# ZulutionAI/MoviiGen1.1

Measured on AMD Instinct MI355X. Metric: denoise-steps/sec, higher is better.
Workload: dtype bf16; 1 GPU; 14B T2V 1920x832x81f bf16 (the metric's configuration; BASELINE configs[2] shape); layers=40, parallelism=single, solver=unipc, weights=random N(0,0.02) bf16, seed 0

## Files before the change

### moviigen1.1_amd/csrc/attn_hd128.hip

```cpp
#include "common.h"
#include "../../include/moviigen_hip.h"

#define ATT_QB 256

__global__ __launch_bounds__(256) void pack_kv_kernel(const uint16_t* __restrict__ k, int64_t ldk,
                                                      const uint16_t* __restrict__ v, int64_t ldv, int64_t L,
                                                      uint16_t* __restrict__ kp, uint16_t* __restrict__ vp, int nt,
                                                      int korder) {
    __shared__ uint16_t tile[64][128 + 8];
    const int head = blockIdx.y, t = blockIdx.x;
    const int64_t k0 = (int64_t)t * 64;
    const int64_t tbase = ((int64_t)head * nt + t) * 8192;
    if (k) {
#pragma unroll
        for (int i = 0; i < 4; ++i) {
            const int id = threadIdx.x + i * 256;
            const int r = id >> 4, c = id & 15;
            u16x8_t u = {0, 0, 0, 0, 0, 0, 0, 0};
            if (k0 + r < L) u = *(const u16x8_t*)(k + (k0 + r) * ldk + head * 128 + c * 8);
            const int row = korder ? ((r & 32) | ((r & 4) << 2) | ((r & 24) >> 1) | (r & 3)) : r;
            *(u16x8_t*)(kp + tbase + c * 512 + row * 8) = u;
        }
    }
    if (v) {
#pragma unroll
        for (int i = 0; i < 4; ++i) {
            const int id = threadIdx.x + i * 256;
            const int r = id >> 4, c = id & 15;
            u16x8_t u = {0, 0, 0, 0, 0, 0, 0, 0};
            if (k0 + r < L) u = *(const u16x8_t*)(v + (k0 + r) * ldv + head * 128 + c * 8);
            *(u16x8_t*)&tile[r][c * 8] = u;
        }
        __syncthreads();
#pragma unroll
        for (int i = 0; i < 4; ++i) {
            const int id = threadIdx.x + i * 256;
            const int kc = id >> 7, d = id & 127;
            u16x8_t u;
#pragma unroll
            for (int j = 0; j < 8; ++j) u[j] = tile[kc * 8 + j][d];
            *(u16x8_t*)(vp + tbase + kc * 1024 + d * 8) = u;
        }
    }
}

#ifdef MG_AB_BUILD
int mg_attn_w64_launch(const uint16_t* q, int64_t ldq, const uint16_t* kp, const uint16_t* vp, uint16_t* o, int64_t ldo,
                       int64_t Lq, int64_t Lk, int heads, float c_log2, int nqb, float* lse, hipStream_t st);
#endif
int mg_attn_m16_launch(const uint16_t* q, int64_t ldq, const uint16_t* kp, const uint16_t* vp, uint16_t* o, int64_t ldo,
                       int64_t Lq, int64_t Lk, int heads, float c_log2, int prescaled, int nqb, float* lse, int reserve_cus,
                       unsigned* workspace, hipStream_t st);

#ifdef MG_AB_BUILD
static int g_attn_variant = 0;
extern "C" int mg_attn_set_variant(int v) {
    if (v != 0 && v != 3) return MG_ERR_ARG;
    g_attn_variant = v;
    return MG_OK;
}
#else
static constexpr int g_attn_variant = 0;
#endif

extern "C" int mg_pack_kv_bf16(const uint16_t* k, int64_t ldk, const uint16_t* v, int64_t ldv, int64_t L, int heads,
                               int head_dim, uint16_t* kp, uint16_t* vp, void* stream) {
    if ((!k && !v) || (k && !kp) || (v && !vp)) return MG_ERR_ARG;
    if (head_dim != 128 || heads <= 0 || L <= 0 || (k && (ldk & 7)) || (v && (ldv & 7))) return MG_ERR_SHAPE;
    const int nt = (int)((L + 63) / 64);
    hipLaunchKernelGGL(pack_kv_kernel, dim3(nt, heads), dim3(256), 0, (hipStream_t)stream, k, ldk, v, ldv, L, kp, vp,
                       nt, g_attn_variant == 3 ? 0 : 1);
    return mg_check_launch();
}

static int attn_fwd_impl(const uint16_t* q, int64_t ldq, const uint16_t* kp, const uint16_t* vp, uint16_t* o, int64_t ldo,
                         float* lse, int64_t Lq, int64_t Lk, int heads, float scale, int prescaled, int reserve_cus, void* workspace,
                         void* stream) {
    if (!q || !kp || !vp || !o) return MG_ERR_ARG;
    if ((uintptr_t)workspace & 7) return MG_ERR_SHAPE;
    if (Lq < 0 || Lk <= 0 || heads <= 0 || reserve_cus < 0) return MG_ERR_SHAPE;
    if ((ldq & 7) || (ldo & 3)) return MG_ERR_SHAPE;
    if (((uintptr_t)q & 15) || ((uintptr_t)kp & 15) || ((uintptr_t)vp & 15) || ((uintptr_t)o & 7)) return MG_ERR_SHAPE;
    if (Lq == 0) return MG_OK;
    const int64_t nqb64 = (Lq + ATT_QB - 1) / ATT_QB;
    if (nqb64 * heads > 0x7fffffffLL) return MG_ERR_SHAPE;
    const int nqb = (int)nqb64;
    const float c_log2 = scale * 1.4426950408889634f;
    hipStream_t st = (hipStream_t)stream;
#ifdef MG_AB_BUILD
    if (g_attn_variant == 3)
        return mg_attn_w64_launch(q, ldq, kp, vp, o, ldo, Lq, Lk, heads, prescaled ? 1.0f : c_log2, nqb, lse, st);
#endif
    return mg_attn_m16_launch(q, ldq, kp, vp, o, ldo, Lq, Lk, heads, c_log2, prescaled, nqb, lse, reserve_cus, (unsigned*)workspace, st);
}

extern "C" int64_t mg_attn_workspace_bytes(void) { return 256; }

extern "C" int mg_attn_fwd_bf16_hd128_lse(const uint16_t* q, int64_t ldq, const uint16_t* kp, const uint16_t* vp,
                                          uint16_t* o, int64_t ldo, float* lse, int64_t Lq, int64_t Lk, int heads,
                                          float scale, void* workspace, void* stream) {
    return attn_fwd_impl(q, ldq, kp, vp, o, ldo, lse, Lq, Lk, heads, scale, 0, 0, workspace, stream);
}
extern "C" int mg_attn_fwd_bf16_hd128(const uint16_t* q, int64_t ldq, const uint16_t* kp, const uint16_t* vp,
                                      uint16_t* o, int64_t ldo, int64_t Lq, int64_t Lk, int heads, float scale,
                                      void* workspace, void* stream) {
    return attn_fwd_impl(q, ldq, kp, vp, o, ldo, nullptr, Lq, Lk, heads, scale, 0, 0, workspace, stream);
}
extern "C" int mg_attn_fwd_bf16_hd128_prescaled(const uint16_t* q, int64_t ldq, const uint16_t* kp, const uint16_t* vp,
                                                uint16_t* o, int64_t ldo, float* lse, int64_t Lq, int64_t Lk, int heads,
                                                int reserve_cus, void* workspace, void* stream) {
    return attn_fwd_impl(q, ldq, kp, vp, o, ldo, lse, Lq, Lk, heads, 1.0f, 1, reserve_cus, workspace, stream);
}
```

### moviigen1.1_amd/csrc/attn_hd128_w64.hip

```cpp
#include <type_traits>
#include "common.h"
#include "../../include/moviigen_hip.h"

#define W64_THREADS 256
#define W64_QB 256
#define W64_TILE 16384
#define W64_K(slot) ((slot) * W64_TILE)
#define W64_V(slot) (3 * W64_TILE + (slot) * W64_TILE)

MG_DEV bf16x8_t w64_bf(u32x4_t v) { return __builtin_bit_cast(bf16x8_t, v); }

struct W64State {
    f32x16_t ot[4][2];
    f32x16_t st[2][2];
    bf16x8_t pf[2][2][2];
    float m_run[2], l_run[2];
    int bad;
};

template <int OFF>
MG_DEV void w64_rd(bf16x8_t& dst, unsigned addr) {
    asm volatile("ds_read_b128 %0, %1 offset:%2" : "=v"(dst) : "v"(addr), "i"(OFF));
}
template <int N>
MG_DEV void w64_wait() {
    asm volatile("s_waitcnt lgkmcnt(%0)" ::"i"(N) : "memory");
}
MG_DEV void w64_mfma_s0(f32x16_t& acc, const bf16x8_t& a, const bf16x8_t& b) {
    asm volatile("v_mfma_f32_32x32x16_bf16 %0, %1, %2, 0" : "=&v"(acc) : "v"(a), "v"(b));
}
MG_DEV void w64_mfma_s(f32x16_t& acc, const bf16x8_t& a, const bf16x8_t& b) {
    asm volatile("v_mfma_f32_32x32x16_bf16 %0, %1, %2, %0" : "+v"(acc) : "v"(a), "v"(b));
}
MG_DEV void w64_mfma_s_after_valu(f32x16_t& acc, const bf16x8_t& a, const bf16x8_t& b) {
    asm volatile("s_nop 7\n\ts_nop 7\n\tv_mfma_f32_32x32x16_bf16 %0, %1, %2, %0" : "+v"(acc) : "v"(a), "v"(b));
}
constexpr int w64_koff(int i) { return i * 2048; }
constexpr int w64_voff(int i) { return (i >> 2) * 4096 + (i & 3) * 512; }

template <int KB>
MG_DEV void w64_softmax_exact(W64State& s, float c_log2) {
#pragma unroll
    for (int qb = 0; qb < 2; ++qb) {
        float tmax = s.st[KB][qb][0];
#pragma unroll
        for (int r = 1; r < 16; ++r) tmax = fmaxf(tmax, s.st[KB][qb][r]);
        tmax = fmaxf(tmax, __shfl_xor(tmax, 32, 64));
        const float m_new = fmaxf(s.m_run[qb], tmax);
        const float mc = m_new * c_log2;
        float psum = 0.f;
        float p[16];
#pragma unroll
        for (int r = 0; r < 16; ++r) {
            p[r] = __builtin_amdgcn_exp2f(s.st[KB][qb][r] * c_log2 - mc);
            psum += p[r];
        }
#pragma unroll
        for (int h = 0; h < 2; ++h) {
            u32x4_t w;
#pragma unroll
            for (int e = 0; e < 4; ++e) w[e] = pack_bf2(p[h * 8 + 2 * e], p[h * 8 + 2 * e + 1]);
            s.pf[KB][qb][h] = w64_bf(w);
        }
        const float alpha = __builtin_amdgcn_exp2f((s.m_run[qb] - m_new) * c_log2);
        s.l_run[qb] = s.l_run[qb] * alpha + psum;
#pragma unroll
        for (int d = 0; d < 4; ++d)
#pragma unroll
            for (int e = 0; e < 16; ++e) s.ot[d][qb][e] *= alpha;
        s.m_run[qb] = m_new;
    }
}

template <int KB>
MG_DEV void w64_mask_init(W64State& s, int lim, int g) {
#pragma unroll
    for (int qb = 0; qb < 2; ++qb)
#pragma unroll
        for (int r = 0; r < 16; ++r) {
            const int key = KB * 32 + (r >> 3) * 16 + g * 8 + (r & 7);
            s.st[KB][qb][r] = key >= lim ? -1e30f : 0.f;
        }
}

template <int KB, int SMODE, bool PV, bool SM, typename Dma>
MG_DEV void w64_step(W64State& s, const bf16x8_t (&qf)[2][8], bf16x8_t (&kf)[4], bf16x8_t (&vf)[4], unsigned lds_k,
                     unsigned lds_v, unsigned nk, unsigned nv, float c_log2, Dma dma) {
    constexpr int SB = 1 - KB;
#ifndef W64_PK_ADD
#define W64_PK_ADD 0
#endif
    float mc[2], psa[2] = {0.f, 0.f}, psb[2] = {0.f, 0.f};
    f32x2_t ps2[2] = {{0.f, 0.f}, {0.f, 0.f}};
    u32x4_t w[2][2];
    if (SM) {
        mc[0] = s.m_run[0] * c_log2;
        mc[1] = s.m_run[1] * c_log2;
    }
    float pa = 0.f, pb = 0.f;
    auto pair_a = [&](int i, int half) __attribute__((always_inline)) {
        if (SM) {
            const int qb = i >> 2, j = (i & 3) * 2 + half;
            pa = __builtin_amdgcn_exp2f(s.st[SB][qb][2 * j] * c_log2 - mc[qb]);
            pb = __builtin_amdgcn_exp2f(s.st[SB][qb][2 * j + 1] * c_log2 - mc[qb]);
            asm volatile("" : "+v"(pa), "+v"(pb));
        }
    };
    auto pair_b = [&](int i, int half) __attribute__((always_inline)) {
        if (SM) {
            const int qb = i >> 2, j = (i & 3) * 2 + half;
#if W64_PK_ADD
            asm volatile("v_pk_add_f32 %0, %0, %1" : "+v"(ps2[qb]) : "v"(__builtin_shufflevector((f32x2_t){pa, pa}, (f32x2_t){pb, pb}, 0, 2)));
            unsigned pk = pack_bf2(pa, pb);
            asm volatile("" : "+v"(pk));
#else
            psa[qb] += pa;
            psb[qb] += pb;
            unsigned pk = pack_bf2(pa, pb);
            asm volatile("" : "+v"(pk), "+v"(psa[qb]), "+v"(psb[qb]));
#endif
            w[qb][j >> 2][j & 3] = pk;
        }
    };
#pragma unroll
    for (int i = 0; i < 8; ++i) {
        const int r = i & 3, r2 = (i + 2) & 3;
        w64_wait<2>();
        __builtin_amdgcn_sched_barrier(0);
        if (SMODE == 1 && i == 0) w64_mfma_s0(s.st[KB][0], kf[r], qf[0][i]);
        else if (SMODE == 2 && i == 0) w64_mfma_s_after_valu(s.st[KB][0], kf[r], qf[0][i]);
        else if (SMODE != 0) w64_mfma_s(s.st[KB][0], kf[r], qf[0][i]);
        __builtin_amdgcn_sched_barrier(0);
        pair_a(i, 0);
        __builtin_amdgcn_sched_barrier(0);
        if (PV) s.ot[i & 3][0] = __builtin_amdgcn_mfma_f32_32x32x16_bf16(vf[r], s.pf[KB][0][i >> 2], s.ot[i & 3][0], 0, 0, 0);
        __builtin_amdgcn_sched_barrier(0);
        pair_b(i, 0);
        __builtin_amdgcn_sched_barrier(0);
        if (SMODE == 1 && i == 0) w64_mfma_s0(s.st[KB][1], kf[r], qf[1][i]);
        else if (SMODE == 2 && i == 0) w64_mfma_s_after_valu(s.st[KB][1], kf[r], qf[1][i]);
        else if (SMODE != 0) w64_mfma_s(s.st[KB][1], kf[r], qf[1][i]);
        __builtin_amdgcn_sched_barrier(0);
        if (SMODE == 0) asm volatile("" ::"v"(kf[r2]));
        if (i < 6) {
            switch (i) {
                case 0: w64_rd<w64_koff(2)>(kf[r2], lds_k); break;
                case 1: w64_rd<w64_koff(3)>(kf[r2], lds_k); break;
                case 2: w64_rd<w64_koff(4)>(kf[r2], lds_k); break;
                case 3: w64_rd<w64_koff(5)>(kf[r2], lds_k); break;
                case 4: w64_rd<w64_koff(6)>(kf[r2], lds_k); break;
                default: w64_rd<w64_koff(7)>(kf[r2], lds_k); break;
            }
        } else if (i == 6) w64_rd<w64_koff(0)>(kf[r2], nk);
        else w64_rd<w64_koff(1)>(kf[r2], nk);
        pair_a(i, 1);
        dma(i);
        __builtin_amdgcn_sched_barrier(0);
        if (PV) s.ot[i & 3][1] = __builtin_amdgcn_mfma_f32_32x32x16_bf16(vf[r], s.pf[KB][1][i >> 2], s.ot[i & 3][1], 0, 0, 0);
        __builtin_amdgcn_sched_barrier(0);
        if (i < 6) {
            switch (i) {
                case 0: w64_rd<w64_voff(2)>(vf[r2], lds_v); break;
                case 1: w64_rd<w64_voff(3)>(vf[r2], lds_v); break;
                case 2: w64_rd<w64_voff(4)>(vf[r2], lds_v); break;
                case 3: w64_rd<w64_voff(5)>(vf[r2], lds_v); break;
                case 4: w64_rd<w64_voff(6)>(vf[r2], lds_v); break;
                default: w64_rd<w64_voff(7)>(vf[r2], lds_v); break;
            }
        } else if (i == 6) w64_rd<w64_voff(0)>(vf[r2], nv);
        else w64_rd<w64_voff(1)>(vf[r2], nv);
        pair_b(i, 1);
        __builtin_amdgcn_sched_barrier(0);
    }
    if (SM) {
#pragma unroll
        for (int qb = 0; qb < 2; ++qb) {
            const float psum = W64_PK_ADD ? ps2[qb][0] + ps2[qb][1] : psa[qb] + psb[qb];
            s.bad |= !(psum <= 1.2676506e30f);
            s.l_run[qb] += psum;
            s.pf[SB][qb][0] = w64_bf(w[qb][0]);
            s.pf[SB][qb][1] = w64_bf(w[qb][1]);
        }
    }
}

struct W64NoDma {
    __device__ __forceinline__ void operator()(int) const {}
};

template <bool PROF>
__global__ __launch_bounds__(W64_THREADS, 1) void attn_hd128_w64_kernel(
    const uint16_t* __restrict__ q, int64_t ldq, const uint16_t* __restrict__ kp, const uint16_t* __restrict__ vp,
    uint16_t* __restrict__ o, int64_t ldo, int64_t Lq, int64_t Lk, int heads, float c_log2, int nqb, int dbg, unsigned long long* __restrict__ prof, float* __restrict__ lse,
    unsigned* __restrict__ flagcnt) {
    __shared__ __attribute__((aligned(16))) char smem[6 * W64_TILE];
    const int bid = blockIdx.x;
    const int tid = threadIdx.x;
    const int wave = __builtin_amdgcn_readfirstlane(tid >> 6);
    const int lane = tid & 63, l31 = lane & 31, g = lane >> 5;
    const int total_items = nqb * heads;
    const int nwg = gridDim.x;
    int item, item_end, item_step;
    if (nwg == total_items) {
        item = bid, item_end = bid + 1, item_step = 1;
    } else {
        const int xcd = bid & 7, slot = bid >> 3;
        item = (int)((int64_t)xcd * total_items / 8) + slot;
        item_end = (int)((int64_t)(xcd + 1) * total_items / 8);
        item_step = nwg >> 3;
    }
    for (; item < item_end; item += item_step) {
    const int head = item / nqb;
    const int qb0 = item - head * nqb;
    __syncthreads();

    bf16x8_t qf[2][8];
    const int64_t qrow_base = (int64_t)qb0 * W64_QB + wave * 64 + l31;
#pragma unroll
    for (int b = 0; b < 2; ++b) {
        const int64_t qr = qrow_base + b * 32;
        const int64_t qrow = qr < Lq ? qr : Lq - 1;
        const uint16_t* qp = q + qrow * ldq + head * 128 + g * 8;
#pragma unroll
        for (int kk = 0; kk < 8; ++kk) qf[b][kk] = w64_bf(*(const u32x4_t*)(qp + kk * 16));
    }
    const int T = (int)((Lk + 63) / 64);
    const int last_lim = (int)(Lk - (int64_t)(T - 1) * 64);
    const char* k_src = (const char*)(kp + ((int64_t)head * T) * 8192 + wave * 2048);
    const char* v_src = (const char*)(vp + ((int64_t)head * T) * 8192 + wave * 2048);
    const unsigned lane_off = lane * 16;
    const int nfull = last_lim == 64 ? T : T - 1;
#ifndef W64_ROTATE
#define W64_ROTATE 0
#endif
    int rot = (!W64_ROTATE || nwg == total_items || nfull < 3) ? 0 : (int)((int64_t)(bid >> 3) * nfull / (nwg >> 3));
    auto phys = [&](int t) __attribute__((always_inline)) {
        if (t >= nfull) return t;
        const int u = t + rot;
        return u < nfull ? u : u - nfull;
    };
    const unsigned lds0 = (unsigned)(uintptr_t)(mg_lptr_t)smem;
    auto dma_k = [&](int t, int slot, int n) __attribute__((always_inline)) {
        const int tt = t < T ? t : T - 1;
        mg_glds16(k_src + ((int64_t)phys(tt) * 16384 + n * 1024) + lane_off, smem + W64_K(slot) + wave * 4096 + n * 1024);
    };
    auto dma_v = [&](int t, int slot, int n) __attribute__((always_inline)) {
        const int tt = t < T ? t : T - 1;
        mg_glds16(v_src + ((int64_t)phys(tt) * 16384 + n * 1024) + lane_off, smem + W64_V(slot) + wave * 4096 + n * 1024);
    };
    const int kperm = (l31 & 0x13) | ((l31 & 4) << 1) | ((l31 & 8) >> 1);
    const unsigned kbase = lds0 + g * 1024 + kperm * 16;
    const unsigned vbase = lds0 + 3 * W64_TILE + g * 2048 + l31 * 16;
    auto k_addr = [&](int slot, int kb) __attribute__((always_inline)) { return kbase + slot * W64_TILE + kb * 512; };
    auto v_addr = [&](int slot, int kb) __attribute__((always_inline)) { return vbase + slot * W64_TILE + kb * 8192; };

    W64State s;
    bf16x8_t kf[4], vf[4];
    auto reset = [&]() __attribute__((always_inline)) {
#pragma unroll
        for (int d = 0; d < 4; ++d)
#pragma unroll
            for (int b = 0; b < 2; ++b)
#pragma unroll
                for (int e = 0; e < 16; ++e) s.ot[d][b][e] = 0.f;
        s.m_run[0] = s.m_run[1] = -1e30f;
        s.l_run[0] = s.l_run[1] = 0.f;
        s.bad = 0;
    };
    reset();
#pragma unroll
    for (int b = 0; b < 2; ++b)
#pragma unroll
        for (int kk = 0; kk < 8; ++kk) asm volatile("" : "+v"(qf[b][kk]));
    auto fence = [&]() __attribute__((always_inline)) {
        asm volatile("s_waitcnt vmcnt(0)" ::: "memory");
        __syncthreads();
    };
    auto prefetch = [&](unsigned ak, unsigned av) __attribute__((always_inline)) {
        w64_rd<w64_koff(0)>(kf[0], ak);
        w64_rd<w64_voff(0)>(vf[0], av);
        w64_rd<w64_koff(1)>(kf[1], ak);
        w64_rd<w64_voff(1)>(vf[1], av);
    };
    auto bare_S = [&](auto kbc, int slot, int lim) __attribute__((always_inline)) {
        constexpr int KB = decltype(kbc)::value;
        if (lim < 64) w64_mask_init<KB>(s, lim, g);
        else {
#pragma unroll
            for (int e = 0; e < 16; ++e) s.st[KB][0][e] = 0.f, s.st[KB][1][e] = 0.f;
        }
        const char* base = smem + W64_K(slot) + g * 1024 + kperm * 16 + KB * 512;
#pragma unroll
        for (int kk = 0; kk < 8; ++kk) {
            const bf16x8_t f = *(const bf16x8_t*)(base + kk * 2048);
            s.st[KB][0] = __builtin_amdgcn_mfma_f32_32x32x16_bf16(f, qf[0][kk], s.st[KB][0], 0, 0, 0);
            s.st[KB][1] = __builtin_amdgcn_mfma_f32_32x32x16_bf16(f, qf[1][kk], s.st[KB][1], 0, 0, 0);
        }
    };
    auto bare_PV = [&](auto kbc, int slot) __attribute__((always_inline)) {
        constexpr int KB = decltype(kbc)::value;
        const char* base = smem + W64_V(slot) + g * 2048 + l31 * 16 + KB * 8192;
#pragma unroll
        for (int i = 0; i < 8; ++i) {
            const bf16x8_t f = *(const bf16x8_t*)(base + w64_voff(i));
            s.ot[i & 3][0] = __builtin_amdgcn_mfma_f32_32x32x16_bf16(f, s.pf[KB][0][i >> 2], s.ot[i & 3][0], 0, 0, 0);
            s.ot[i & 3][1] = __builtin_amdgcn_mfma_f32_32x32x16_bf16(f, s.pf[KB][1][i >> 2], s.ot[i & 3][1], 0, 0, 0);
        }
    };
    using KB0 = std::integral_constant<int, 0>;
    using KB1 = std::integral_constant<int, 1>;

    bool exact_pass = nfull < 3;
    if (!exact_pass) {
#pragma unroll
        for (int n = 0; n < 4; ++n) dma_k(0, 0, n), dma_v(0, 0, n), dma_k(1, 1, n);
        fence();
#pragma unroll
        for (int n = 0; n < 4; ++n) dma_k(2, 2, n), dma_v(1, 1, n);
        bare_S(KB0{}, 0, 64);
        w64_softmax_exact<0>(s, c_log2);
        bare_S(KB1{}, 0, 64);
        prefetch(k_addr(1, 0), v_addr(0, 0));
        w64_step<0, 1, true, true>(s, qf, kf, vf, k_addr(1, 0), v_addr(0, 0), k_addr(1, 1), v_addr(0, 1), c_log2, W64NoDma());
        int s0 = 0, s1 = 1, s2 = 2;
        int t = 1;
        unsigned long long pf_fence = 0, pf_a = 0, pf_b = 0, pf_n = 0;
        for (; t + 1 < nfull; ++t) {
            const unsigned long long c0 = PROF ? __builtin_amdgcn_s_memtime() : 0;
            fence();
            const unsigned long long c1 = PROF ? __builtin_amdgcn_s_memtime() : 0;
            w64_step<1, 1, true, true>(s, qf, kf, vf, k_addr(s1, 1), v_addr(s0, 1), k_addr(s2, 0), v_addr(s1, 0), c_log2,
                                       [&](int n) __attribute__((always_inline)) {
                                           if (n < 4) dma_k(t + 2, s0, n);
                                           else dma_v(t + 1, s2, n - 4);
                                       });
            const unsigned long long c2 = PROF ? __builtin_amdgcn_s_memtime() : 0;
            w64_step<0, 1, true, true>(s, qf, kf, vf, k_addr(s2, 0), v_addr(s1, 0), k_addr(s2, 1), v_addr(s1, 1), c_log2,
                                       W64NoDma());
            if (PROF) {
                const unsigned long long c3 = __builtin_amdgcn_s_memtime();
                pf_fence += c1 - c0, pf_a += c2 - c1, pf_b += c3 - c2, pf_n += 1;
            }
            const int tmp = s0;
            s0 = s1, s1 = s2, s2 = tmp;
        }
        if (PROF && prof && lane == 0) {
            atomicAdd(prof + wave * 4 + 0, pf_fence);
            atomicAdd(prof + wave * 4 + 1, pf_a);
            atomicAdd(prof + wave * 4 + 2, pf_b);
            atomicAdd(prof + wave * 4 + 3, pf_n);
        }
        fence();
        if (t + 1 < T) {
#pragma unroll
            for (int n = 0; n < 4; ++n) dma_v(t + 1, s2, n);
        }
        w64_step<1, 1, true, true>(s, qf, kf, vf, k_addr(s1, 1), v_addr(s0, 1), k_addr(s2, 0), v_addr(s1, 0), c_log2, W64NoDma());
        if (t + 1 < T) {
            w64_mask_init<0>(s, last_lim, g);
            w64_step<0, 2, true, true>(s, qf, kf, vf, k_addr(s2, 0), v_addr(s1, 0), k_addr(s2, 1), v_addr(s1, 1), c_log2, W64NoDma());
            fence();
            w64_mask_init<1>(s, last_lim, g);
            w64_step<1, 2, true, true>(s, qf, kf, vf, k_addr(s2, 1), v_addr(s1, 1), 0, v_addr(s2, 0), c_log2, W64NoDma());
            w64_step<0, 0, true, true>(s, qf, kf, vf, 0, v_addr(s2, 0), 0, v_addr(s2, 1), c_log2, W64NoDma());
            w64_step<1, 0, true, false>(s, qf, kf, vf, 0, v_addr(s2, 1), 0, 0, c_log2, W64NoDma());
        } else {
            w64_step<0, 0, true, true>(s, qf, kf, vf, 0, v_addr(s1, 0), 0, v_addr(s1, 1), c_log2, W64NoDma());
            w64_step<1, 0, true, false>(s, qf, kf, vf, 0, v_addr(s1, 1), 0, 0, c_log2, W64NoDma());
        }
        w64_wait<0>();
        asm volatile("" ::"v"(kf[0]), "v"(kf[1]), "v"(kf[2]), "v"(kf[3]), "v"(vf[0]), "v"(vf[1]), "v"(vf[2]), "v"(vf[3]));
        exact_pass = __syncthreads_or(s.bad) != 0;
        if (exact_pass && flagcnt && tid == 0) atomicAdd(flagcnt, 1u);
        if (dbg & 1) exact_pass = false;
    }
    if (exact_pass) {
        reset();
        rot = 0;
        for (int t = 0; t < T; ++t) {
            __syncthreads();
#pragma unroll
            for (int n = 0; n < 4; ++n) dma_k(t, 0, n), dma_v(t, 0, n);
            fence();
            const int lim = t == T - 1 ? last_lim : 64;
            bare_S(KB0{}, 0, lim);
            bare_S(KB1{}, 0, lim);
            w64_softmax_exact<0>(s, c_log2);
            bare_PV(KB0{}, 0);
            w64_softmax_exact<1>(s, c_log2);
            bare_PV(KB1{}, 0);
        }
    }

#pragma unroll
    for (int b = 0; b < 2; ++b) {
        const float l_tot = s.l_run[b] + __shfl_xor(s.l_run[b], 32, 64);
        const float inv = 1.f / l_tot;
        const int64_t qr = (int64_t)qb0 * W64_QB + wave * 64 + l31 + b * 32;
        if (lse && g == 0 && qr < Lq) lse[(int64_t)head * Lq + qr] = (s.m_run[b] * c_log2 + __log2f(l_tot)) * 0.6931471805599453f;
        if (qr < Lq) {
            uint16_t* op = o + qr * ldo + head * 128 + g * 4;
#pragma unroll
            for (int d = 0; d < 4; ++d)
#pragma unroll
                for (int rq = 0; rq < 4; ++rq) {
                    uint2 pk;
                    pk.x = pack_bf2(s.ot[d][b][rq * 4 + 0] * inv, s.ot[d][b][rq * 4 + 1] * inv);
                    pk.y = pack_bf2(s.ot[d][b][rq * 4 + 2] * inv, s.ot[d][b][rq * 4 + 3] * inv);
                    *(uint2*)(op + d * 32 + rq * 8) = pk;
                }
        }
    }
    }
}

static int g_w64_dbg = 0;
static unsigned long long* g_w64_prof = nullptr;
static unsigned* g_w64_flagcnt = nullptr;
void mg_attn_m16_hooks(int dbg, unsigned long long* prof, unsigned* flagcnt);
static void w64_sync_hooks() { mg_attn_m16_hooks(g_w64_dbg, g_w64_prof, g_w64_flagcnt); }
extern "C" void mg_attn_w64_profile(unsigned long long* dev_buf) { g_w64_prof = dev_buf; w64_sync_hooks(); }
extern "C" void mg_attn_w64_debug(int flags) { g_w64_dbg = flags; w64_sync_hooks(); }
extern "C" void mg_attn_w64_flag_counter(unsigned* dev_counter) { g_w64_flagcnt = dev_counter; w64_sync_hooks(); }

int mg_attn_w64_launch(const uint16_t* q, int64_t ldq, const uint16_t* kp, const uint16_t* vp, uint16_t* o, int64_t ldo,
                       int64_t Lq, int64_t Lk, int heads, float c_log2, int nqb, float* lse, hipStream_t st) {
    const int n_cu = mg_persistent_cus();
    if (n_cu < 0) return MG_ERR_LAUNCH;
    const int total = nqb * heads;
    const unsigned grid = total <= n_cu ? (unsigned)total : (unsigned)n_cu;
    if (g_w64_prof)
        hipLaunchKernelGGL((attn_hd128_w64_kernel<true>), dim3(grid), dim3(W64_THREADS), 0, st, q, ldq, kp, vp, o, ldo, Lq, Lk,
                           heads, c_log2, nqb, g_w64_dbg, g_w64_prof, lse, g_w64_flagcnt);
    else
        hipLaunchKernelGGL((attn_hd128_w64_kernel<false>), dim3(grid), dim3(W64_THREADS), 0, st, q, ldq, kp, vp, o, ldo, Lq, Lk,
                           heads, c_log2, nqb, g_w64_dbg, nullptr, lse, g_w64_flagcnt);
    return mg_check_launch();
}
```

Baseline: 0.04686 steps/s.

## Add 8-wave attention kernel for short key sequences

```diff
diff --git a/moviigen1.1_amd/csrc/attn_hd128.hip b/moviigen1.1_amd/csrc/attn_hd128.hip
--- a/moviigen1.1_amd/csrc/attn_hd128.hip
+++ b/moviigen1.1_amd/csrc/attn_hd128.hip
@@ -51,11 +51,15 @@
 int mg_attn_m16_launch(const uint16_t* q, int64_t ldq, const uint16_t* kp, const uint16_t* vp, uint16_t* o, int64_t ldo,
                        int64_t Lq, int64_t Lk, int heads, float c_log2, int prescaled, int nqb, float* lse, int reserve_cus,
                        unsigned* workspace, hipStream_t st);
+int mg_attn_m16w8_launch(const uint16_t* q, int64_t ldq, const uint16_t* kp, const uint16_t* vp, uint16_t* o, int64_t ldo,
+                         int64_t Lq, int64_t Lk, int heads, float c_log2, int prescaled, int nqb, unsigned* workspace, hipStream_t st);
+
+#define ATT_K_SHORT 1024
 
 #ifdef MG_AB_BUILD
 static int g_attn_variant = 0;
 extern "C" int mg_attn_set_variant(int v) {
-    if (v != 0 && v != 3) return MG_ERR_ARG;
+    if (v != 0 && v != 3 && v != 5 && v != 6) return MG_ERR_ARG;
     g_attn_variant = v;
     return MG_OK;
 }
@@ -91,6 +95,9 @@
     if (g_attn_variant == 3)
         return mg_attn_w64_launch(q, ldq, kp, vp, o, ldo, Lq, Lk, heads, prescaled ? 1.0f : c_log2, nqb, lse, st);
 #endif
+    const bool is_short = g_attn_variant == 6 || (g_attn_variant != 5 && Lk <= ATT_K_SHORT);
+    if (is_short && !lse && reserve_cus == 0)
+        return mg_attn_m16w8_launch(q, ldq, kp, vp, o, ldo, Lq, Lk, heads, c_log2, prescaled, nqb, (unsigned*)workspace, st);
     return mg_attn_m16_launch(q, ldq, kp, vp, o, ldo, Lq, Lk, heads, c_log2, prescaled, nqb, lse, reserve_cus, (unsigned*)workspace, st);
 }
 
diff --git a/moviigen1.1_amd/csrc/attn_hd128_m16w8.hip b/moviigen1.1_amd/csrc/attn_hd128_m16w8.hip
--- /dev/null
+++ b/moviigen1.1_amd/csrc/attn_hd128_m16w8.hip
@@ -0,0 +1,569 @@
+#include <type_traits>
+#include "common.h"
+#include "../../include/moviigen_hip.h"
+
+#define P8_THREADS 512
+#define P8_NQ 2
+#define P8_QB 256
+#define P8_TILE 16384
+#define P8_K(slot) ((slot) * P8_TILE)
+#define P8_V(slot) (3 * P8_TILE + (slot) * P8_TILE)
+
+MG_DEV bf16x8_t p8_bf(u32x4_t v) { return __builtin_bit_cast(bf16x8_t, v); }
+struct P8State {
+    f32x4_t ot[8][P8_NQ];
+    f32x4_t st[2][2][P8_NQ];
+    bf16x8_t pf[2][P8_NQ];
+    f32x4_t mq[P8_NQ];
+    float m_run[P8_NQ], l_run[P8_NQ];
+    float psa[P8_NQ], psb[P8_NQ];
+    int bad;
+};
+
+template <int OFF>
+MG_DEV void p8_rd(bf16x8_t& dst, unsigned addr) {
+    asm volatile("ds_read_b128 %0, %1 offset:%2" : "=v"(dst) : "v"(addr), "i"(OFF));
+}
+template <int OFF>
+MG_DEV void p8_rdk(bf16x8_t& dst, unsigned addr) {
+    asm volatile("ds_read_b128 %0, %1 offset:%2" : "=a"(dst) : "v"(addr), "i"(OFF));
+}
+template <int N>
+MG_DEV void p8_wait() {
+    asm volatile("s_waitcnt lgkmcnt(%0)" ::"i"(N) : "memory");
+}
+MG_DEV void p8_mfma_s0(f32x4_t& acc, const bf16x8_t& a, const bf16x8_t& b, const f32x4_t& c) {
+    asm volatile("v_mfma_f32_16x16x32_bf16 %0, %1, %2, %3" : "=&v"(acc) : "a"(a), "a"(b), "v"(c));
+}
+MG_DEV void p8_mfma_s(f32x4_t& acc, const bf16x8_t& a, const bf16x8_t& b) {
+    asm volatile("v_mfma_f32_16x16x32_bf16 %0, %1, %2, %0" : "+v"(acc) : "a"(a), "a"(b));
+}
+MG_DEV void p8_mfma_s_after_valu(f32x4_t& acc, const bf16x8_t& a, const bf16x8_t& b) {
+    asm volatile("s_nop 7\n\ts_nop 7\n\tv_mfma_f32_16x16x32_bf16 %0, %1, %2, %0" : "+v"(acc) : "a"(a), "a"(b));
+}
+constexpr int p8_koff(int i) { return (i >> 2) * 256 + (i & 3) * 4096; }
+constexpr int p8_voff(int i) { return i * 256; }
+
+template <int KB>
+MG_DEV void p8_softmax_exact(P8State& s, float c) {
+#pragma unroll
+    for (int n = 0; n < P8_NQ; ++n) {
+        float tmax = s.st[KB][0][n][0];
+#pragma unroll
+        for (int r = 1; r < 4; ++r) tmax = fmaxf(tmax, s.st[KB][0][n][r]);
+#pragma unroll
+        for (int r = 0; r < 4; ++r) tmax = fmaxf(tmax, s.st[KB][1][n][r]);
+        tmax = fmaxf(tmax, __shfl_xor(tmax, 16, 64));
+        tmax = fmaxf(tmax, __shfl_xor(tmax, 32, 64));
+        const float m_new = fmaxf(s.m_run[n], tmax);
+        float psum = 0.f;
+        float p[8];
+#pragma unroll
+        for (int r = 0; r < 8; ++r) {
+            p[r] = __builtin_amdgcn_exp2f((s.st[KB][r >> 2][n][r & 3] - m_new) * c);
+            psum += p[r];
+        }
+        u32x4_t w;
+#pragma unroll
+        for (int e = 0; e < 4; ++e) w[e] = pack_bf2(p[2 * e], p[2 * e + 1]);
+        s.pf[KB][n] = p8_bf(w);
+        const float alpha = __builtin_amdgcn_exp2f((s.m_run[n] - m_new) * c);
+        s.l_run[n] = s.l_run[n] * alpha + psum;
+#pragma unroll
+        for (int d = 0; d < 8; ++d)
+#pragma unroll
+            for (int e = 0; e < 4; ++e) s.ot[d][n][e] *= alpha;
+        s.m_run[n] = m_new;
+    }
+}
+
+template <int KB>
+MG_DEV void p8_softmax_zero(P8State& s, float c) {
+#pragma unroll
+    for (int n = 0; n < P8_NQ; ++n) {
+        float psum = 0.f;
+        float p[8];
+#pragma unroll
+        for (int r = 0; r < 8; ++r) {
+            p[r] = __builtin_amdgcn_exp2f(s.st[KB][r >> 2][n][r & 3] * c);
+            psum += p[r];
+        }
+        u32x4_t w;
+#pragma unroll
+        for (int e = 0; e < 4; ++e) w[e] = pack_bf2(p[2 * e], p[2 * e + 1]);
+        s.pf[KB][n] = p8_bf(w);
+        s.l_run[n] += psum;
+    }
+}
+
+template <int KB>
+MG_DEV void p8_mask_init(P8State& s, int lim, int G, const f32x4_t (&base)[P8_NQ]) {
+#pragma unroll
+    for (int blk = 0; blk < 2; ++blk)
+#pragma unroll
+        for (int n = 0; n < P8_NQ; ++n)
+#pragma unroll
+            for (int r = 0; r < 4; ++r) {
+                const int key = KB * 32 + G * 8 + blk * 4 + r;
+                s.st[KB][blk][n][r] = key >= lim ? -1e30f : base[n][0];
+            }
+}
+
+template <int KB, int SMODE, bool PV, bool SM, bool SCALED, int LKO = 0, int LVO = 0, int NKO = 0, int NVO = 0, typename Dma>
+MG_DEV void p8_step(P8State& s, const bf16x8_t (&qf)[P8_NQ][4], bf16x8_t (&kf)[4], bf16x8_t (&vf)[4], unsigned lds_k,
+                    unsigned lds_v, unsigned nk, unsigned nv, float c, Dma dma) {
+    constexpr int SB = 1 - KB;
+    u32x4_t w[P8_NQ];
+    float pa = 0.f, pb = 0.f;
+    auto exp_a = [&](int i) __attribute__((always_inline)) {
+        if (SM) {
+            const int n = i >> 2, wd = i & 3;
+            const float x = s.st[SB][wd >> 1][n][(wd & 1) * 2];
+            pa = __builtin_amdgcn_exp2f(SCALED ? x * c : x);
+            asm volatile("" : "+v"(pa));
+        }
+    };
+    auto exp_b = [&](int i) __attribute__((always_inline)) {
+        if (SM) {
+            const int n = i >> 2, wd = i & 3;
+            const float x = s.st[SB][wd >> 1][n][(wd & 1) * 2 + 1];
+            pb = __builtin_amdgcn_exp2f(SCALED ? x * c : x);
+            asm volatile("" : "+v"(pb));
+        }
+    };
+    auto add_cvt = [&](int i) __attribute__((always_inline)) {
+        if (SM) {
+            const int n = i >> 2, wd = i & 3;
+            s.psa[n] += pa;
+            asm volatile("" : "+v"(s.psa[n]));
+            s.psb[n] += pb;
+            asm volatile("" : "+v"(s.psb[n]));
+            unsigned pk = pack_bf2(pa, pb);
+            asm volatile("" : "+v"(pk));
+            w[n][wd] = pk;
+        }
+    };
+    auto S = [&](int i, int n) __attribute__((always_inline)) {
+        const int blk = i >> 2, c = i & 3, r = i & 3;
+        if (SMODE == 1 && c == 0) p8_mfma_s0(s.st[KB][blk][n], kf[r], qf[n][c], s.mq[n]);
+        else if (SMODE == 2 && c == 0) p8_mfma_s_after_valu(s.st[KB][blk][n], kf[r], qf[n][c]);
+        else if (SMODE != 0) p8_mfma_s(s.st[KB][blk][n], kf[r], qf[n][c]);
+    };
+    auto P = [&](int i, int n) __attribute__((always_inline)) {
+        if (PV) s.ot[i][n] = __builtin_amdgcn_mfma_f32_16x16x32_bf16(vf[i & 3], s.pf[KB][n], s.ot[i][n], 0, 0, 0);
+    };
+    auto rdK = [&](int i) __attribute__((always_inline)) {
+        const int r2 = (i + 2) & 3;
+        if (SMODE == 0) asm volatile("" ::"a"(kf[r2]));
+        if (i < 6) {
+            switch (i) {
+                case 0: p8_rdk<p8_koff(2) + LKO>(kf[r2], lds_k); break;
+                case 1: p8_rdk<p8_koff(3) + LKO>(kf[r2], lds_k); break;
+                case 2: p8_rdk<p8_koff(4) + LKO>(kf[r2], lds_k); break;
+                case 3: p8_rdk<p8_koff(5) + LKO>(kf[r2], lds_k); break;
+                case 4: p8_rdk<p8_koff(6) + LKO>(kf[r2], lds_k); break;
+                default: p8_rdk<p8_koff(7) + LKO>(kf[r2], lds_k); break;
+            }
+        } else if (i == 6) p8_rdk<p8_koff(0) + NKO>(kf[r2], nk);
+        else p8_rdk<p8_koff(1) + NKO>(kf[r2], nk);
+    };
+    auto rdV = [&](int i) __attribute__((always_inline)) {
+        const int r2 = (i + 2) & 3;
+        if (i < 6) {
+            switch (i) {
+                case 0: p8_rd<p8_voff(2) + LVO>(vf[r2], lds_v); break;
+                case 1: p8_rd<p8_voff(3) + LVO>(vf[r2], lds_v); break;
+                case 2: p8_rd<p8_voff(4) + LVO>(vf[r2], lds_v); break;
+                case 3: p8_rd<p8_voff(5) + LVO>(vf[r2], lds_v); break;
+                case 4: p8_rd<p8_voff(6) + LVO>(vf[r2], lds_v); break;
+                default: p8_rd<p8_voff(7) + LVO>(vf[r2], lds_v); break;
+            }
+        } else if (i == 6) p8_rd<p8_voff(0) + NVO>(vf[r2], nv);
+        else p8_rd<p8_voff(1) + NVO>(vf[r2], nv);
+    };
+    if (SM) {
+#pragma unroll
+        for (int blk = 0; blk < 2; ++blk)
+#pragma unroll
+            for (int n = 0; n < P8_NQ; ++n) asm volatile("" : "+v"(s.st[SB][blk][n]));
+    }
+#define P8_SB() __builtin_amdgcn_sched_barrier(0)
+#pragma unroll
+    for (int i = 0; i < 8; ++i) {
+        p8_wait<2>();
+        P8_SB();
+        S(i, 0); P8_SB();
+        exp_a(i); P8_SB();
+        S(i, 1); P8_SB();
+        exp_b(i); P8_SB();
+        P(i, 0); P8_SB();
+        add_cvt(i); P8_SB();
+        P(i, 1); P8_SB();
+        rdK(i); P8_SB(); rdV(i); P8_SB();
+        dma(i); P8_SB();
+    }
+#undef P8_SB
+    if (SM) {
+#pragma unroll
+        for (int n = 0; n < P8_NQ; ++n) s.pf[SB][n] = p8_bf(w[n]);
+    }
+}
+
+MG_DEV int p8_lane() {
+    int l;
+    asm volatile("v_mbcnt_lo_u32_b32 %0, -1, 0\n\tv_mbcnt_hi_u32_b32 %0, -1, %0" : "=v"(l));
+    return l;
+}
+
+struct P8NoDma {
+    __device__ __forceinline__ void operator()(int) const {}
+};
+
+template <bool SCALED>
+__global__ __launch_bounds__(P8_THREADS, 1) void attn_hd128_m16w8_kernel(
+    const uint16_t* __restrict__ q, int64_t ldq, const uint16_t* __restrict__ kp, const uint16_t* __restrict__ vp,
+    uint16_t* __restrict__ o, int64_t ldo, int64_t Lq, int64_t Lk, int heads, float c_log2, int nqb, int dbg,
+    unsigned* __restrict__ flagcnt, unsigned* __restrict__ tickets) {
+    __shared__ __attribute__((aligned(16))) char smem[6 * P8_TILE];
+    __shared__ int s_next_item;
+    const int bid = blockIdx.x;
+    const int tid = threadIdx.x;
+    const int wave = __builtin_amdgcn_readfirstlane(tid >> 6);
+    const int total_items = nqb * heads;
+    const int nwg = gridDim.x;
+    const bool ticketed = tickets != nullptr && nwg != total_items;
+    int item, item_end, item_step;
+    if (nwg == total_items || ticketed) {
+        item = bid, item_end = ticketed ? total_items : bid + 1, item_step = 1;
+    } else {
+        const int xcd = bid & 7, slot = bid >> 3;
+        item = (int)((int64_t)xcd * total_items / 8) + slot;
+        item_end = (int)((int64_t)(xcd + 1) * total_items / 8);
+        item_step = nwg >> 3;
+    }
+    unsigned next_ticket = 0;
+    while (item < item_end) {
+    if (ticketed && tid == 0) next_ticket = atomicAdd(tickets, 1u);
+    const int head = item / nqb;
+    const int qb0 = item - head * nqb;
+    const int lane = p8_lane();
+    int qi = lane & 15, G = lane >> 4;
+    __syncthreads();
+
+    bf16x8_t qf[P8_NQ][4];
+    const int64_t qrow_base = (int64_t)qb0 * P8_QB + wave * 32 + qi;
+#pragma unroll
+    for (int n = 0; n < P8_NQ; ++n) {
+        const int64_t qr = qrow_base + n * 16;
+        const int64_t qrow = qr < Lq ? qr : Lq - 1;
+        const uint16_t* qp = q + qrow * ldq + head * 128 + G * 8;
+#pragma unroll
+        for (int c = 0; c < 4; ++c) qf[n][c] = p8_bf(*(const u32x4_t*)(qp + c * 32));
+    }
+    const int T = (int)((Lk + 63) / 64);
+    const int last_lim = (int)(Lk - (int64_t)(T - 1) * 64);
+    const int nfull = last_lim == 64 ? T : T - 1;
+    const unsigned lds0 = (unsigned)(uintptr_t)(mg_lptr_t)smem;
+    const uint64_t kb64 = (uint64_t)(uintptr_t)(kp + ((int64_t)head * T) * 8192), vb64 = (uint64_t)(uintptr_t)(vp + ((int64_t)head * T) * 8192);
+    const u32x4_t rs_k = {(unsigned)__builtin_amdgcn_readfirstlane((int)(unsigned)kb64), (unsigned)__builtin_amdgcn_readfirstlane((int)((unsigned)(kb64 >> 32) & 0xffffu)),
+                          (unsigned)T * P8_TILE, 0x00020000u};
+    const u32x4_t rs_v = {(unsigned)__builtin_amdgcn_readfirstlane((int)(unsigned)vb64), (unsigned)__builtin_amdgcn_readfirstlane((int)((unsigned)(vb64 >> 32) & 0xffffu)),
+                          (unsigned)T * P8_TILE, 0x00020000u};
+    const int dvo = wave * 2048 + lane * 16;
+    const unsigned lds_w = (unsigned)__builtin_amdgcn_readfirstlane((int)(lds0 + wave * 2048));
+    auto dma_tile2 = [&](const u32x4_t& rs, int t, unsigned lbase) __attribute__((always_inline)) {
+        const int soff = __builtin_amdgcn_readfirstlane((t < T ? t : T - 1) * P8_TILE);
+        asm volatile("s_mov_b32 m0, %2\n\ts_nop 4\n\t"
+                     "buffer_load_dwordx4 %0, %1, %3 offen lds\n\t"
+                     "buffer_load_dwordx4 %0, %1, %3 offen offset:1024 lds"
+                     :: "v"(dvo), "s"(rs), "s"(lbase), "s"(soff) : "memory");
+    };
+    auto dma_k2 = [&](int t, int slot) __attribute__((always_inline)) { dma_tile2(rs_k, t, lds_w + P8_K(slot)); };
+    auto dma_v2 = [&](int t, int slot) __attribute__((always_inline)) { dma_tile2(rs_v, t, lds_w + P8_V(slot)); };
+    unsigned kbase = lds0 + G * 1024 + qi * 16;
+    unsigned vbase = lds0 + 3 * P8_TILE + G * 2048 + qi * 16;
+    auto k_addr = [&](int slot, int kb) __attribute__((always_inline)) { return kbase + slot * P8_TILE + kb * 512; };
+    auto v_addr = [&](int slot, int kb) __attribute__((always_inline)) { return vbase + slot * P8_TILE + kb * 8192; };
+
+    P8State s;
+    bf16x8_t kf[4], vf[4];
+    auto reset = [&]() __attribute__((always_inline)) {
+#pragma unroll
+        for (int d = 0; d < 8; ++d)
+#pragma unroll
+            for (int n = 0; n < P8_NQ; ++n) s.ot[d][n] = (f32x4_t){0.f, 0.f, 0.f, 0.f};
+#pragma unroll
+        for (int n = 0; n < P8_NQ; ++n) s.m_run[n] = -1e30f, s.l_run[n] = 0.f, s.psa[n] = 0.f, s.psb[n] = 0.f;
+        s.bad = 0;
+    };
+    reset();
+    auto q_pin = [&]() __attribute__((always_inline)) {
+#pragma unroll
+        for (int n = 0; n < P8_NQ; ++n)
+#pragma unroll
+            for (int c = 0; c < 4; ++c) asm volatile("" : "+a"(qf[n][c]));
+    };
+    auto fence = [&]() __attribute__((always_inline)) {
+        asm volatile("s_waitcnt vmcnt(0)" ::: "memory");
+        __syncthreads();
+    };
+    auto fence_hot = [&]() __attribute__((always_inline)) {
+        asm volatile("s_waitcnt vmcnt(0)\n\ts_barrier" ::: "memory");
+    };
+    auto prefetch = [&](unsigned ak, unsigned av) __attribute__((always_inline)) {
+        p8_rdk<p8_koff(0)>(kf[0], ak);
+        p8_rd<p8_voff(0)>(vf[0], av);
+        p8_rdk<p8_koff(1)>(kf[1], ak);
+        p8_rd<p8_voff(1)>(vf[1], av);
+    };
+    const f32x4_t zero4[P8_NQ] = {{0.f, 0.f, 0.f, 0.f}, {0.f, 0.f, 0.f, 0.f}};
+    auto bare_S = [&](auto kbc, int slot, int lim) __attribute__((always_inline)) {
+        constexpr int KB = decltype(kbc)::value;
+        if (lim < 64) p8_mask_init<KB>(s, lim, G, zero4);
+        else {
+#pragma unroll
+            for (int blk = 0; blk < 2; ++blk)
+#pragma unroll
+                for (int n = 0; n < P8_NQ; ++n) s.st[KB][blk][n] = (f32x4_t){0.f, 0.f, 0.f, 0.f};
+        }
+        const char* base = smem + P8_K(slot) + G * 1024 + qi * 16 + KB * 512;
+#pragma unroll
+        for (int i = 0; i < 8; ++i) {
+            const bf16x8_t f = *(const bf16x8_t*)(base + p8_koff(i));
+#pragma unroll
+            for (int n = 0; n < P8_NQ; ++n)
+                s.st[KB][i >> 2][n] = __builtin_amdgcn_mfma_f32_16x16x32_bf16(f, qf[n][i & 3], s.st[KB][i >> 2][n], 0, 0, 0);
+        }
+    };
+    auto bare_PV = [&](auto kbc, int slot) __attribute__((always_inline)) {
+        constexpr int KB = decltype(kbc)::value;
+        const char* base = smem + P8_V(slot) + G * 2048 + qi * 16 + KB * 8192;
+#pragma unroll
+        for (int i = 0; i < 8; ++i) {
+            const bf16x8_t f = *(const bf16x8_t*)(base + p8_voff(i));
+#pragma unroll
+            for (int n = 0; n < P8_NQ; ++n)
+                s.ot[i][n] = __builtin_amdgcn_mfma_f32_16x16x32_bf16(f, s.pf[KB][n], s.ot[i][n], 0, 0, 0);
+        }
+    };
+    using KB0 = std::integral_constant<int, 0>;
+    using KB1 = std::integral_constant<int, 1>;
+
+    bool exact_pass = nfull < 3;
+    if (!exact_pass) {
+    for (int attempt = 0;; ++attempt) {
+        auto tile_max = [&](float (&mx)[P8_NQ]) __attribute__((always_inline)) {
+#pragma unroll
+            for (int n = 0; n < P8_NQ; ++n) {
+                float a = fmaxf(fmaxf(s.st[0][0][n][0], s.st[0][0][n][1]), fmaxf(s.st[0][0][n][2], s.st[0][0][n][3]));
+                float b = fmaxf(fmaxf(s.st[0][1][n][0], s.st[0][1][n][1]), fmaxf(s.st[0][1][n][2], s.st[0][1][n][3]));
+                float c2 = fmaxf(fmaxf(s.st[1][0][n][0], s.st[1][0][n][1]), fmaxf(s.st[1][0][n][2], s.st[1][0][n][3]));
+                float d2 = fmaxf(fmaxf(s.st[1][1][n][0], s.st[1][1][n][1]), fmaxf(s.st[1][1][n][2], s.st[1][1][n][3]));
+                mx[n] = fmaxf(mx[n], fmaxf(fmaxf(a, b), fmaxf(c2, d2)));
+            }
+        };
+        auto set_reference = [&](const float (&mx)[P8_NQ], float above) __attribute__((always_inline)) {
+#pragma unroll
+            for (int n = 0; n < P8_NQ; ++n) {
+                float m = fmaxf(mx[n], __shfl_xor(mx[n], 16, 64));
+                m = fmaxf(m, __shfl_xor(m, 32, 64)) + above;
+                s.mq[n] = (f32x4_t){-m, -m, -m, -m};
+            }
+        };
+        if (attempt) {
+            float mx[P8_NQ] = {-1e30f, -1e30f};
+#pragma unroll
+            for (int a = 0; a < 4; ++a) dma_k2(a, a);
+            for (int t = 0; t < T; ++t) {
+                asm volatile("s_waitcnt vmcnt(6)" ::: "memory");
+                __syncthreads();
+                dma_k2(t + 4, (t + 4) % 6);
+                const int lim = t == T - 1 ? last_lim : 64;
+                bare_S(KB0{}, t % 6, lim);
+                bare_S(KB1{}, t % 6, lim);
+                tile_max(mx);
+            }
+            asm volatile("s_waitcnt vmcnt(0)" ::: "memory");
+            set_reference(mx, 0.f);
+            __syncthreads();
+            reset();
+        }
+        dma_k2(0, 0), dma_v2(0, 0), dma_k2(1, 1);
+        fence();
+        q_pin();
+        dma_k2(2, 2), dma_v2(1, 1);
+        bare_S(KB0{}, 0, 64);
+        bare_S(KB1{}, 0, 64);
+        if (attempt == 0) {
+            float mx[P8_NQ] = {-1e30f, -1e30f};
+            tile_max(mx);
+            set_reference(mx, c_log2 > 1e-20f ? 64.f / c_log2 : 0.f);
+        }
+#pragma unroll
+        for (int kb = 0; kb < 2; ++kb)
+#pragma unroll
+            for (int blk = 0; blk < 2; ++blk)
+#pragma unroll
+                for (int n = 0; n < P8_NQ; ++n) s.st[kb][blk][n] += s.mq[n];
+        p8_softmax_zero<0>(s, c_log2);
+#pragma unroll
+        for (int n = 0; n < P8_NQ; ++n) asm volatile("" : "+v"(s.l_run[n]));
+        prefetch(k_addr(1, 0), v_addr(0, 0));
+        p8_step<0, 1, true, true, SCALED>(s, qf, kf, vf, k_addr(1, 0), v_addr(0, 0), k_addr(1, 1), v_addr(0, 1), c_log2, P8NoDma());
+        int t = 1;
+        unsigned ka0 = k_addr(0, 0), ka1 = k_addr(1, 0), ka2 = k_addr(2, 0);
+        unsigned va0 = v_addr(0, 0), va1 = v_addr(1, 0), va2 = v_addr(2, 0);
+        unsigned lk0 = (unsigned)__builtin_amdgcn_readfirstlane((int)(lds0 + P8_K(0) + wave * 2048));
+        unsigned lk1 = lk0 + P8_TILE, lk2 = lk0 + 2 * P8_TILE;
+        int offk = (t + 2) * P8_TILE, offv = (t + 1) * P8_TILE;
+        unsigned keep_m0, rot_tmp;
+#define P8_BDMA0(VOFF, RS, SOFF, LBASE, IMM)                                                                                               \
+    asm volatile("s_add_u32 m0, %2, %3\n\ts_nop 0\n\tbuffer_load_dwordx4 %0, %1, %4 offen lds"                                             \
+                 :: "v"(VOFF), "s"(RS), "s"(LBASE), "n"(IMM), "s"(SOFF) : "memory", "scc")
+#define P8_BDMAN(VOFF, RS, SOFF, IMM)                                                                                                      \
+    asm volatile("buffer_load_dwordx4 %0, %1, %3 offen offset:%2 lds" :: "v"(VOFF), "s"(RS), "n"(IMM), "s"(SOFF) : "memory")
+        asm volatile("s_mov_b32 %0, m0\n\ts_nop 4" : "=s"(keep_m0) :: "memory");
+        __builtin_amdgcn_s_waitcnt(0x0F70);
+        asm volatile("" : "+v"(ka0), "+v"(ka1), "+v"(ka2), "+v"(va0), "+v"(va1), "+v"(va2));
+        for (; t + 1 < nfull; ++t) {
+            fence_hot();
+            p8_step<1, 1, true, true, SCALED, 512, 8192, 0, 0>(s, qf, kf, vf, ka1, va0, ka2, va1, c_log2,
+                                       [&](int n) __attribute__((always_inline)) {
+                                           switch (n) {
+                                               case 0: P8_BDMA0(dvo, rs_k, offk, lk0, 0); break;
+                                               case 1: P8_BDMAN(dvo, rs_k, offk, 1024); break;
+                                               case 2: P8_BDMA0(dvo, rs_v, offv, lk2, 3 * P8_TILE); break;
+                                               case 3: P8_BDMAN(dvo, rs_v, offv, 1024); break;
+                                               default: break;
+                                           }
+                                       });
+            p8_step<0, 1, true, true, SCALED, 0, 0, 512, 8192>(s, qf, kf, vf, ka2, va1, ka2, va1, c_log2,
+                                       [&](int n) __attribute__((always_inline)) {
+                                           if (n == 0)
+                                               asm volatile("s_add_u32 %0, %0, 0x4000\n\ts_add_u32 %1, %1, 0x4000" : "+s"(offk), "+s"(offv) : : "scc");
+                                           else if (n == 1)
+                                               asm volatile("s_mov_b32 %3, %0\n\ts_mov_b32 %0, %1\n\ts_mov_b32 %1, %2\n\ts_mov_b32 %2, %3"
+                                                            : "+s"(lk0), "+s"(lk1), "+s"(lk2), "=&s"(rot_tmp));
+                                           else if (n == 7) {
+                                               asm volatile("v_swap_b32 %0, %1\n\tv_swap_b32 %1, %2" : "+v"(ka0), "+v"(ka1), "+v"(ka2));
+                                               asm volatile("v_swap_b32 %0, %1\n\tv_swap_b32 %1, %2" : "+v"(va0), "+v"(va1), "+v"(va2));
+                                           }
+                                       });
+        }
+#undef P8_BDMA0
+#undef P8_BDMAN
+        asm volatile("s_mov_b32 m0, %0" :: "s"(keep_m0) : "memory");
+        static_assert(P8_TILE == 0x4000, "the literal above");
+        const int s0 = (t - 1) % 3, s1 = t % 3, s2 = (t + 1) % 3;
+        {
+            const int l2 = p8_lane();
+            qi = l2 & 15, G = l2 >> 4;
+            kbase = lds0 + G * 1024 + qi * 16;
+            vbase = lds0 + 3 * P8_TILE + G * 2048 + qi * 16;
+        }
+        fence();
+        if (t + 1 < T) {
+            dma_v2(t + 1, s2);
+        }
+        p8_step<1, 1, true, true, SCALED>(s, qf, kf, vf, k_addr(s1, 1), v_addr(s0, 1), k_addr(s2, 0), v_addr(s1, 0), c_log2, P8NoDma());
+        int sl = s1;
+        if (t + 1 < T) {
+            p8_mask_init<0>(s, last_lim, G, s.mq);
+            p8_step<0, 2, true, true, SCALED>(s, qf, kf, vf, k_addr(s2, 0), v_addr(s1, 0), k_addr(s2, 1), v_addr(s1, 1), c_log2, P8NoDma());
+            fence();
+            p8_mask_init<1>(s, last_lim, G, s.mq);
+            p8_step<1, 2, true, true, SCALED>(s, qf, kf, vf, k_addr(s2, 1), v_addr(s1, 1), k_addr(s2, 1), v_addr(s2, 0), c_log2, P8NoDma());
+            sl = s2;
+        }
+        p8_step<0, 0, true, true, SCALED>(s, qf, kf, vf, k_addr(sl, 1), v_addr(sl, 0), k_addr(sl, 1), v_addr(sl, 1), c_log2, P8NoDma());
+        p8_step<1, 0, true, false, SCALED>(s, qf, kf, vf, k_addr(sl, 1), v_addr(sl, 1), k_addr(sl, 1), v_addr(sl, 1), c_log2, P8NoDma());
+        p8_wait<0>();
+        asm volatile("" ::"a"(kf[0]), "a"(kf[1]), "a"(kf[2]), "a"(kf[3]), "v"(vf[0]), "v"(vf[1]), "v"(vf[2]), "v"(vf[3]));
+#pragma unroll
+        for (int n = 0; n < P8_NQ; ++n) {
+            s.l_run[n] += s.psa[n] + s.psb[n];
+            s.psa[n] = s.psb[n] = 0.f;
+            float lt = s.l_run[n] + __shfl_xor(s.l_run[n], 16, 64);
+            lt += __shfl_xor(lt, 32, 64);
+            s.bad |= !(lt >= 8.4703295e-22f && lt <= 1.2379400e27f);
+        }
+        const bool flagged = __syncthreads_or(s.bad) != 0;
+        if (!flagged || (dbg & 1)) break;
+        if (flagcnt && tid == 0) atomicAdd(flagcnt + (attempt ? 1 : 0), 1u);
+        if (attempt) {
+            exact_pass = true;
+            break;
+        }
+    }
+    }
+    if (exact_pass) {
+        reset();
+        for (int t = 0; t < T; ++t) {
+            __syncthreads();
+            dma_k2(t, 0), dma_v2(t, 0);
+            fence();
+            q_pin();
+            const int lim = t == T - 1 ? last_lim : 64;
+            bare_S(KB0{}, 0, lim);
+            bare_S(KB1{}, 0, lim);
+            p8_softmax_exact<0>(s, c_log2);
+            bare_PV(KB0{}, 0);
+            p8_softmax_exact<1>(s, c_log2);
+            bare_PV(KB1{}, 0);
+        }
+    }
+
+    {
+        const int l3 = p8_lane();
+        qi = l3 & 15, G = l3 >> 4;
+    }
+#pragma unroll
+    for (int n = 0; n < P8_NQ; ++n) {
+        float l_tot = s.l_run[n] + __shfl_xor(s.l_run[n], 16, 64);
+        l_tot += __shfl_xor(l_tot, 32, 64);
+        const float inv = 1.f / l_tot;
+        const int64_t qr = (int64_t)qb0 * P8_QB + wave * 32 + n * 16 + qi;
+        if (qr < Lq) {
+            uint16_t* op = o + qr * ldo + head * 128 + G * 4;
+#pragma unroll
+            for (int d = 0; d < 8; ++d) {
+                uint2 pk;
+                pk.x = pack_bf2(s.ot[d][n][0] * inv, s.ot[d][n][1] * inv);
+                pk.y = pack_bf2(s.ot[d][n][2] * inv, s.ot[d][n][3] * inv);
+                *(uint2*)(op + d * 16) = pk;
+            }
+        }
+    }
+    if (ticketed) {
+        if (tid == 0) s_next_item = nwg + (int)next_ticket;
+        __syncthreads();
+        item = __builtin_amdgcn_readfirstlane(s_next_item);
+    } else
+        item += item_step;
+    }
+    if (ticketed && tid == 0 && atomicAdd(tickets + 1, 1u) == (unsigned)nwg - 1) {
+        __hip_atomic_store(tickets, 0u, __ATOMIC_RELAXED, __HIP_MEMORY_SCOPE_AGENT);
+        __hip_atomic_store(tickets + 1, 0u, __ATOMIC_RELAXED, __HIP_MEMORY_SCOPE_AGENT);
+    }
+}
+
+static int g_p8_dbg = 0;
+static unsigned* g_p8_flagcnt = nullptr;
+void mg_attn_m16w8_hooks(int dbg, unsigned* flagcnt) { g_p8_dbg = dbg, g_p8_flagcnt = flagcnt; }
+
+int mg_attn_m16w8_launch(const uint16_t* q, int64_t ldq, const uint16_t* kp, const uint16_t* vp, uint16_t* o, int64_t ldo,
+                         int64_t Lq, int64_t Lk, int heads, float c_log2, int prescaled, int nqb, unsigned* workspace, hipStream_t st) {
+    const int n_cu = mg_persistent_cus(0);
+    if (n_cu < 0) return MG_ERR_LAUNCH;
+    const int total = nqb * heads;
+    const unsigned grid = total <= n_cu ? (unsigned)total : (unsigned)n_cu;
+    unsigned* tickets = nullptr;
+    if (workspace && (int64_t)total >= 32 * (int64_t)grid && !(g_p8_dbg & 16)) tickets = workspace;
+    if (prescaled)
+        hipLaunchKernelGGL((attn_hd128_m16w8_kernel<false>), dim3(grid), dim3(P8_THREADS), 0, st, q, ldq, kp, vp, o, ldo, Lq, Lk, heads, 1.0f, nqb,
+                           g_p8_dbg, g_p8_flagcnt, tickets);
+    else
+        hipLaunchKernelGGL((attn_hd128_m16w8_kernel<true>), dim3(grid), dim3(P8_THREADS), 0, st, q, ldq, kp, vp, o, ldo, Lq, Lk, heads, c_log2, nqb,
+                           g_p8_dbg, g_p8_flagcnt, tickets);
+    return mg_check_launch();
+}
diff --git a/moviigen1.1_amd/csrc/attn_hd128_w64.hip b/moviigen1.1_amd/csrc/attn_hd128_w64.hip
--- a/moviigen1.1_amd/csrc/attn_hd128_w64.hip
+++ b/moviigen1.1_amd/csrc/attn_hd128_w64.hip
@@ -418,7 +418,8 @@
 static unsigned long long* g_w64_prof = nullptr;
 static unsigned* g_w64_flagcnt = nullptr;
 void mg_attn_m16_hooks(int dbg, unsigned long long* prof, unsigned* flagcnt);
-static void w64_sync_hooks() { mg_attn_m16_hooks(g_w64_dbg, g_w64_prof, g_w64_flagcnt); }
+void mg_attn_m16w8_hooks(int dbg, unsigned* flagcnt);
+static void w64_sync_hooks() { mg_attn_m16_hooks(g_w64_dbg, g_w64_prof, g_w64_flagcnt), mg_attn_m16w8_hooks(g_w64_dbg, g_w64_flagcnt); }
 extern "C" void mg_attn_w64_profile(unsigned long long* dev_buf) { g_w64_prof = dev_buf; w64_sync_hooks(); }
 extern "C" void mg_attn_w64_debug(int flags) { g_w64_dbg = flags; w64_sync_hooks(); }
 extern "C" void mg_attn_w64_flag_counter(unsigned* dev_counter) { g_w64_flagcnt = dev_counter; w64_sync_hooks(); }
```

Measured after the change: 0.04690 steps/s (median of 6 runs). No clear change (+0.1%).
